# imatge-upc/rsis

Measured on AMD Instinct MI355X. Metric: training images/sec at 256x256, T=10, batch=32 per GPU, higher is better.
Workload: dtype f32

## Files before the change

rsis_amd/csrc/conv_wgrad_tiled.hip:

```cpp
#include "common.h"
#include "limb_split.h"
#include <stdlib.h>
#include <string.h>

typedef __attribute__((address_space(3))) void* lds_vp_t;
typedef __bf16 wg_bf16x8 __attribute__((ext_vector_type(8)));
typedef unsigned wg_u32x4 __attribute__((ext_vector_type(4)));

#define WG_LIMB_PRODUCTS 6
[[maybe_unused]] __device__ constexpr int wg_limb_pa[9] = {2, 1, 0, 1, 0, 0, 2, 1, 2};
[[maybe_unused]] __device__ constexpr int wg_limb_pb[9] = {0, 1, 2, 0, 1, 0, 1, 2, 2};

__device__ __forceinline__ void wg_limb_pack8(const float (&v)[8], wg_bf16x8 (&out)[3]) {
  wg_u32x4 q[3];
#pragma unroll
  for (int m = 0; m < 4; ++m) {
    float lo[3], hi[3];
    rsis_limb_split3(v[2 * m], lo[0], lo[1], lo[2]);
    rsis_limb_split3(v[2 * m + 1], hi[0], hi[1], hi[2]);
    q[0][m] = __builtin_amdgcn_perm(__float_as_uint(v[2 * m + 1]), __float_as_uint(v[2 * m]), 0x07060302u);
    q[1][m] = __builtin_amdgcn_perm(__float_as_uint(hi[1]), __float_as_uint(lo[1]), 0x07060302u);
    q[2][m] = __builtin_amdgcn_perm(__float_as_uint(hi[2]), __float_as_uint(lo[2]), 0x07060302u);
  }
#pragma unroll
  for (int l = 0; l < 3; ++l) out[l] = __builtin_bit_cast(wg_bf16x8, q[l]);
}

struct WgradTiledArgs {
  const float* dy;
  const float* x;
  float* dw;
  int B, Cs, H, W, Cout;
  int ldo, n_off, interleave_hid;
  int n_co_tiles, n_n_tiles, n_sp_tiles, tiles_per_split;
};

#define RSIS_OOB 0x7FFFFFF0u

template <int BM, int BN, int WGM, int WGN, int KS, int TW, int KSP = 1, int RAG = 0, int LIMB = 0>
__device__ __forceinline__ void wgrad_tiled_body(const WgradTiledArgs& p, const int bx, const int by) {
#if __HIP_DEVICE_COMPILE__
  constexpr int TM = BM / WGM / 32, TN = BN / WGN / 32;
  constexpr int KK = KS * KS, HALO = KS / 2;
  constexpr int TP = KS == 1 ? 32 : 64;
  constexpr int TH = TP / TW;
  constexpr int NG = TP / 4;
  constexpr int GPR = TW / 4;
  constexpr int PW = TW + 2 * HALO, PH = TH + 2 * HALO, IMS = PW * PH;
  constexpr int CI_P = KS == 1 ? BN : (BN + KK - 2) / KK + 1;
  constexpr int AS = BM * TP;
  constexpr int XS = KS == 1 ? BN * TP : (CI_P * IMS + 255) / 256 * 256;
  constexpr int NA = BM * NG / 256;
  constexpr int NB4 = KS == 1 ? BN * NG / 256 : 0;
  constexpr int NB1 = KS == 1 ? 0 : XS / 256;
  static_assert(WGM * WGN * KSP == 4 && (BM * NG) % 256 == 0 && (KS == 3 || (BN * NG) % 256 == 0) && (NG / 2) % KSP == 0 && (NG / 2 / KSP) % 2 == 0, "config");

  __shared__ __attribute__((aligned(16))) float lds[2 * (AS + XS)];
  float* const As0 = lds;
  float* const Xs0 = lds + 2 * AS;

  const int tid = threadIdx.x, lane = tid & 63, l31 = lane & 31, hi = lane >> 5;
  const int wave = __builtin_amdgcn_readfirstlane(tid >> 6);
  const int wk = wave / (WGM * WGN), wm = (wave % (WGM * WGN)) / WGN, wn = wave % WGN;
  const int H = p.H, W = p.W, HW = H * W, Cs = p.Cs, Cout = p.Cout;
  const int co_t = bx % p.n_co_tiles, n_t = bx / p.n_co_tiles;
  const int co0 = co_t * BM, n0 = n_t * BN;
  const int ci0 = n0 / KK;
  const int Nn = Cs * KK;
  const int tiles_x = RAG ? (W + TW - 1) / TW : W / TW, tiles_y = RAG ? (H + TH - 1) / TH : H / TH;
  const int rx = W - (tiles_x - 1) * TW, ry = H - (tiles_y - 1) * TH;
  const int t_begin = by * p.tiles_per_split;
  const int t_end = min(t_begin + p.tiles_per_split, p.n_sp_tiles);
  if (t_begin >= t_end) return;

  unsigned voa[NA];
#pragma unroll
  for (int i = 0; i < NA; ++i) {
    const int idx = tid + i * 256;
    const int row = idx / NG, sl = idx % NG;
    const int G = (sl & ~7) | ((sl & 7) ^ (row & 7));
    const int y = G / GPR, x4 = G % GPR;
    voa[i] = co0 + row < Cout ? ((unsigned)((co0 + row) * HW + y * W + x4 * 4) * 4u) | (RAG == 2 && x4 * 4 >= rx ? 1u : 0u) | (RAG == 2 && y >= ry ? 2u : 0u) : RSIS_OOB;
  }
  unsigned voa1[RAG == 1 ? 4 * NA : 1];
  unsigned vob1r[RAG == 1 && NB4 ? 4 * NB4 : 1];
  if constexpr (RAG == 1) {
#pragma unroll
    for (int k = 0; k < 4 * NA; ++k) {
      const int P = k * 256 + tid, idx = P >> 2, e = P & 3;
      const int row = idx / NG, sl = idx % NG;
      const int G = (sl & ~7) | ((sl & 7) ^ (row & 7));
      const int y = G / GPR, x = (G % GPR) * 4 + e;
      voa1[k] = co0 + row < Cout ? ((unsigned)((co0 + row) * HW + y * W + x) * 4u) | (x >= rx ? 1u : 0u) | (y >= ry ? 2u : 0u) : RSIS_OOB;
    }
    if constexpr (KS == 1) {
#pragma unroll
      for (int k = 0; k < 4 * NB4; ++k) {
        const int P = k * 256 + tid, idx = P >> 2, e = P & 3;
        const int row = idx / NG, sl = idx % NG;
        const int G = (sl & ~7) | ((sl & 7) ^ (row & 7));
        const int y = G / GPR, x = (G % GPR) * 4 + e;
        vob1r[k] = n0 + row < Cs ? ((unsigned)((n0 + row) * HW + y * W + x) * 4u) | (x >= rx ? 1u : 0u) | (y >= ry ? 2u : 0u) : RSIS_OOB;
      }
    }
  }
  unsigned vob4[NB4 ? NB4 : 1];
  unsigned vob1[NB1 ? NB1 : 1];
  unsigned cls1[NB1 ? NB1 : 1];
  if constexpr (KS == 1) {
#pragma unroll
    for (int i = 0; i < NB4; ++i) {
      const int idx = tid + i * 256;
      const int row = idx / NG, sl = idx % NG;
      const int G = (sl & ~7) | ((sl & 7) ^ (row & 7));
      const int y = G / GPR, x4 = G % GPR;
      vob4[i] = n0 + row < Cs ? ((unsigned)((n0 + row) * HW + y * W + x4 * 4) * 4u) | (RAG == 2 && x4 * 4 >= rx ? 1u : 0u) | (RAG == 2 && y >= ry ? 2u : 0u) : RSIS_OOB;
    }
  } else {
#pragma unroll
    for (int i = 0; i < NB1; ++i) {
      const int e = tid + i * 256;
      const int cl = e / IMS, rem = e - cl * IMS;
      const int py = rem / PW, pxx = rem - py * PW;
      const bool ok = cl < CI_P && ci0 + cl < Cs;
      vob1[i] = ok ? (unsigned)(cl * HW + py * W + pxx) * 4u : RSIS_OOB;
      cls1[i] = (py == 0 ? 1u : 0u) | (py - 1 >= ry ? 2u : 0u) | (pxx == 0 ? 4u : 0u) | (pxx - 1 >= rx ? 8u : 0u);
    }
  }

  int sg[NG / 2 / KSP];
  int bo[NG / 2 / KSP];
#pragma unroll
  for (int gg = 0; gg < NG / 2 / KSP; ++gg) {
    const int g = gg * KSP + (KSP == 1 ? 0 : wk);
    sg[gg] = ((2 * g + hi) ^ (l31 & 7)) * 4;
    bo[gg] = KS == 1 ? 0 : (g / (TW / 8)) * PW + (g % (TW / 8)) * 8;
  }
  const int arow = (wm * TM * 32 + l31) * TP;
  int xb[TN];
#pragma unroll
  for (int j = 0; j < TN; ++j) {
    const int nl = wn * TN * 32 + j * 32 + l31;
    if constexpr (KS == 1) {
      xb[j] = nl * TP;
    } else {
      const int n = n0 + nl;
      const int cl = n / KK - ci0, rs = n - (n / KK) * KK;
      xb[j] = cl * IMS + (rs / KS) * PW + (rs % KS) + 4 * hi;
    }
  }

  f32x16 acc[TM][TN];
#pragma unroll
  for (int i = 0; i < TM; ++i)
#pragma unroll
    for (int j = 0; j < TN; ++j)
#pragma unroll
      for (int r = 0; r < 16; ++r) acc[i][j][r] = 0.f;

  int tb = t_begin / (tiles_x * tiles_y);
  int trem = t_begin - tb * (tiles_x * tiles_y);
  int ty = trem / tiles_x, tx = trem - ty * tiles_x;

#define WG_ISSUE(BUF)                                                                                          \
  {                                                                                                            \
    const int y0 = ty * TH, x0 = tx * TW;                                                                      \
    const float* ab = p.dy + ((size_t)tb * Cout * HW + y0 * W + x0);                                           \
    const __amdgpu_buffer_rsrc_t ra_ = __builtin_amdgcn_make_buffer_rsrc((void*)ab, 0, 0x7FFFFFF0, 0x00020000); \
    const unsigned lastm = (tx == tiles_x - 1 ? 1u : 0u) | (ty == tiles_y - 1 ? 2u : 0u);                      \
    if constexpr (RAG == 1) {                                                                                  \
      float* As = As0 + (BUF) * AS + wave * 64;                                                                \
      _Pragma("unroll") for (int k = 0; k < 4 * NA; ++k)                                                       \
        __builtin_amdgcn_raw_ptr_buffer_load_lds(ra_, (lds_vp_t)(As + k * 256), 4, (voa1[k] & lastm) ? RSIS_OOB : (voa1[k] & ~3u), 0, 0, 0); \
    } else {                                                                                                   \
      float* As = As0 + (BUF) * AS + wave * 256;                                                               \
      _Pragma("unroll") for (int i = 0; i < NA; ++i)                                                           \
        __builtin_amdgcn_raw_ptr_buffer_load_lds(ra_, (lds_vp_t)(As + i * 1024), 16,                           \
                                                 RAG == 2 ? ((voa[i] & lastm) ? RSIS_OOB : (voa[i] & ~3u)) : voa[i], 0, 0, 0); \
    }                                                                                                          \
    if constexpr (KS == 1) {                                                                                   \
      const float* bb = p.x + ((size_t)tb * Cs * HW + y0 * W + x0);                                            \
      const __amdgpu_buffer_rsrc_t rb_ = __builtin_amdgcn_make_buffer_rsrc((void*)bb, 0, 0x7FFFFFF0, 0x00020000); \
      if constexpr (RAG == 1) {                                                                                \
        float* Xs = Xs0 + (BUF) * XS + wave * 64;                                                              \
        _Pragma("unroll") for (int k = 0; k < 4 * NB4; ++k)                                                    \
          __builtin_amdgcn_raw_ptr_buffer_load_lds(rb_, (lds_vp_t)(Xs + k * 256), 4, (vob1r[k] & lastm) ? RSIS_OOB : (vob1r[k] & ~3u), 0, 0, 0); \
      } else {                                                                                                 \
        float* Xs = Xs0 + (BUF) * XS + wave * 256;                                                             \
        _Pragma("unroll") for (int i = 0; i < NB4; ++i)                                                        \
          __builtin_amdgcn_raw_ptr_buffer_load_lds(rb_, (lds_vp_t)(Xs + i * 1024), 16,                         \
                                                   RAG == 2 ? ((vob4[i] & lastm) ? RSIS_OOB : (vob4[i] & ~3u)) : vob4[i], 0, 0, 0); \
      }                                                                                                        \
    } else {                                                                                                   \
      const float* bb = p.x + (((size_t)tb * Cs + ci0) * HW + (y0 - 1) * W + (x0 - 1));                        \
      const __amdgpu_buffer_rsrc_t rb_ = __builtin_amdgcn_make_buffer_rsrc((void*)bb, 0, 0x7FFFFFF0, 0x00020000); \
      const unsigned edge = (y0 == 0 ? 1u : 0u) | (ty == tiles_y - 1 ? 2u : 0u) | (x0 == 0 ? 4u : 0u) | (tx == tiles_x - 1 ? 8u : 0u); \
      float* Xs = Xs0 + (BUF) * XS + wave * 64;                                                                \
      _Pragma("unroll") for (int i = 0; i < NB1; ++i) {                                                        \
        const unsigned vo = (cls1[i] & edge) ? RSIS_OOB : vob1[i];                                             \
        __builtin_amdgcn_raw_ptr_buffer_load_lds(rb_, (lds_vp_t)(Xs + i * 256), 4, vo, 0, 0, 0);               \
      }                                                                                                        \
    }                                                                                                          \
    if (++tx == tiles_x) { tx = 0; if (++ty == tiles_y) { ty = 0; ++tb; } }                                    \
  }
#define WG_LAND() __builtin_amdgcn_s_waitcnt(0x0F70);

  WG_ISSUE(0)
  WG_LAND()
  __syncthreads();
  const int ntl = t_end - t_begin;
  for (int t = 0; t < ntl; ++t) {
    const int cur = t & 1;
    if (t + 1 < ntl) WG_ISSUE(cur ^ 1)
    {
      const float* As = As0 + cur * AS + arow;
      const float* Xs = Xs0 + cur * XS;
      if constexpr (LIMB) {
#pragma unroll
        for (int g = 0; g < NG / 2 / KSP; g += 2) {
          wg_bf16x8 al[TM][3], bl[TN][3];
#pragma unroll
          for (int i = 0; i < TM; ++i) {
            const f32x4 a0 = *reinterpret_cast<const f32x4*>(As + i * 32 * TP + sg[g]);
            const f32x4 a1 = *reinterpret_cast<const f32x4*>(As + i * 32 * TP + sg[g + 1]);
            const float v[8] = {a0[0], a0[1], a0[2], a0[3], a1[0], a1[1], a1[2], a1[3]};
            wg_limb_pack8(v, al[i]);
          }
#pragma unroll
          for (int j = 0; j < TN; ++j) {
            float v[8];
            if constexpr (KS == 1) {
              const f32x4 b0 = *reinterpret_cast<const f32x4*>(Xs + xb[j] + sg[g]);
              const f32x4 b1 = *reinterpret_cast<const f32x4*>(Xs + xb[j] + sg[g + 1]);
#pragma unroll
              for (int e = 0; e < 4; ++e) { v[e] = b0[e]; v[4 + e] = b1[e]; }
            } else {
#pragma unroll
              for (int u = 0; u < 2; ++u)
#pragma unroll
                for (int e = 0; e < 4; ++e)
                  v[4 * u + e] = Xs[xb[j] + (KSP == 1 ? ((g + u) / (TW / 8)) * PW + ((g + u) % (TW / 8)) * 8 : bo[g + u]) + e];
            }
            wg_limb_pack8(v, bl[j]);
          }
#pragma unroll
          for (int q = 0; q < WG_LIMB_PRODUCTS; ++q)
#pragma unroll
            for (int i = 0; i < TM; ++i)
#pragma unroll
              for (int j = 0; j < TN; ++j)
                acc[i][j] = __builtin_amdgcn_mfma_f32_32x32x16_bf16(al[i][wg_limb_pa[q]], bl[j][wg_limb_pb[q]], acc[i][j], 0, 0, 0);
        }
      } else
#pragma unroll
      for (int g = 0; g < NG / 2 / KSP; ++g) {
        f32x4 a4[TM];
#pragma unroll
        for (int i = 0; i < TM; ++i) a4[i] = *reinterpret_cast<const f32x4*>(As + i * 32 * TP + sg[g]);
        if constexpr (KS == 1) {
          f32x4 b4[TN];
#pragma unroll
          for (int j = 0; j < TN; ++j) b4[j] = *reinterpret_cast<const f32x4*>(Xs + xb[j] + sg[g]);
#pragma unroll
          for (int e = 0; e < 4; ++e)
#pragma unroll
            for (int i = 0; i < TM; ++i)
#pragma unroll
              for (int j = 0; j < TN; ++j) acc[i][j] = __builtin_amdgcn_mfma_f32_32x32x2f32(a4[i][e], b4[j][e], acc[i][j], 0, 0, 0);
        } else {
#pragma unroll
          for (int e = 0; e < 4; ++e) {
            float b[TN];
#pragma unroll
            for (int j = 0; j < TN; ++j) b[j] = Xs[xb[j] + (KSP == 1 ? (g / (TW / 8)) * PW + (g % (TW / 8)) * 8 : bo[g]) + e];
#pragma unroll
            for (int i = 0; i < TM; ++i)
#pragma unroll
              for (int j = 0; j < TN; ++j) acc[i][j] = __builtin_amdgcn_mfma_f32_32x32x2f32(a4[i][e], b[j], acc[i][j], 0, 0, 0);
          }
        }
      }
    }
    WG_LAND()
    __syncthreads();
  }
#undef WG_ISSUE
#undef WG_LAND

  const __amdgpu_buffer_rsrc_t rdw = __builtin_amdgcn_make_buffer_rsrc((void*)p.dw, 0, (unsigned)((size_t)Cout * p.ldo * 4), 0x00020000);
  const int ihid = p.interleave_hid;
  const unsigned ldb = (unsigned)p.ldo * 4u;
#pragma unroll
  for (int j = 0; j < TN; ++j) {
    const int n = n0 + wn * TN * 32 + j * 32 + l31;
    if (n >= Nn) continue;
#pragma unroll
    for (int i = 0; i < TM; ++i) {
      const int row0 = co0 + wm * TM * 32 + i * 32 + 4 * hi;
      const int rows_left = Cout - row0;
      const unsigned vo = (unsigned)((ihid > 0 ? row0 >> 2 : row0) * p.ldo + p.n_off + n) * 4u;
#pragma unroll
      for (int r = 0; r < 16; ++r) {
        const int k = (r & 3) + 8 * (r >> 2);
        const unsigned ro = (unsigned)(ihid > 0 ? (r & 3) * ihid + 2 * (r >> 2) : k) * ldb;
        __builtin_amdgcn_raw_ptr_buffer_atomic_fadd_f32(acc[i][j][r], rdw, k < rows_left ? vo + ro : 0x7FFFFFF0u, 0, 0);
      }
    }
  }
#endif
}

#define RSIS_WG_MAXJ 48
struct WgradTiledGroup {
  int n;
  int begin[RSIS_WG_MAXJ + 1];
  WgradTiledArgs job[RSIS_WG_MAXJ];
};
static_assert(sizeof(WgradTiledGroup) <= 4000, "kernel arguments are limited to 4 KB");

template <int BM, int BN, int WGM, int WGN, int KS, int TW, int KSP = 1, int RAG = 0, int LIMB = 0>
__global__ __launch_bounds__(256) void conv_wgrad_tiled_group_kernel(const WgradTiledGroup g) {
  const int b = blockIdx.x;
  int lo = 0, hi = g.n - 1;
  while (lo < hi) {
    const int mid = (lo + hi + 1) >> 1;
    if (g.begin[mid] <= b) lo = mid; else hi = mid - 1;
  }
  const WgradTiledArgs& p = g.job[lo];
  const int local = b - g.begin[lo];
  const int ntile = p.n_co_tiles * p.n_n_tiles;
  wgrad_tiled_body<BM, BN, WGM, WGN, KS, TW, KSP, RAG, LIMB>(p, local % ntile, local / ntile);
}

static unsigned wg_limb_mask(int ks, int tw) {
  if (ks == 3) return tw == 16 ? 0x3Fu : (tw == 8 ? 1u << 5 : 0u);
  return tw == 16 || tw == 8 ? 1u << 2 : 0u;
}
static bool wg_use_limbs(int ks, int tw, int code, int rag) {
  static const int mode = [] {
    const char* e = getenv("RSIS_WGRAD_LIMBS");
    if (!e || !e[0]) return 0;
    if (e[0] == '0') return 1;
    return strcmp(e, "all") == 0 ? 2 : 0;
  }();
  if (mode) return mode == 2;
  return rag == 0 && ((wg_limb_mask(ks, tw) >> code) & 1u);
}

static int tiled_tw(int H, int W, int ks) {
  const int tp = ks == 1 ? 32 : 64;
  for (int tw = ks == 1 ? 32 : 16; tw >= 8; tw >>= 1)
    if (W % tw == 0 && H % (tp / tw) == 0) return tw;
  return 0;
}
static int tiled_tw_ragged(int W, int ks) {
  const int wide = ks == 1 ? 32 : 16;
  return W > 16 ? wide : (W > 8 ? 16 : 8);
}

static int tiled_cfg_code(const WgradTiledArgs& a, int ks) {
  const int nmod = (a.Cs * ks * ks) % 128;
  const bool narrow = nmod != 0 && nmod <= 64;
  if (ks == 1 && a.Cout > 32) return 2;
  if (a.Cout <= 32) return narrow && !rsis_deterministic() ? 0 : 1;
  if (a.Cout <= 64) return narrow ? 2 : 3;
  return narrow ? 4 : 5;
}

static void tiled_split_plan(WgradTiledArgs* jobs, int n, int ks, bool big_tile, bool alone, int rag) {
  if (alone && rag == 0) {
    WgradTiledArgs& a = jobs[0];
    const int ntile = a.n_co_tiles * a.n_n_tiles;
    const int slots = ks == 1 ? (big_tile ? 256 : 512) : 256 * (big_tile ? 2 : 3);
    int nsplit = ntile >= slots ? 1 : slots / ntile;
    if (nsplit > a.n_sp_tiles / 2) nsplit = a.n_sp_tiles / 2;
    if (nsplit < 1 || rsis_deterministic()) nsplit = 1;
    a.tiles_per_split = rsis_cdiv(a.n_sp_tiles, nsplit);
    return;
  }
  long total_iters = 0;
  for (int j = 0; j < n; ++j) total_iters += (long)jobs[j].n_co_tiles * jobs[j].n_n_tiles * jobs[j].n_sp_tiles;
  static const int env_tb = getenv("RSIS_WG_GROUP_BLOCKS") ? atoi(getenv("RSIS_WG_GROUP_BLOCKS")) : 0;
  const long target_blocks = env_tb > 0 ? env_tb : 2048;
  long L = (total_iters + target_blocks - 1) / target_blocks;
  if (L < 2) L = 2;
  if (rsis_deterministic()) L = 1L << 40;
  for (int j = 0; j < n; ++j) {
    int nsplit = rsis_cdiv(jobs[j].n_sp_tiles, L);
    if (nsplit < 1) nsplit = 1;
    jobs[j].tiles_per_split = rsis_cdiv(jobs[j].n_sp_tiles, nsplit);
  }
}

template <int BM, int BN, int WGM, int WGN, int KS, int TW, int KSP = 1, int RAG = 0, int LIMB = 0>
static int launch_group_cfg(WgradTiledArgs* jobs, int n, bool alone, hipStream_t st) {
  constexpr int TH = (KS == 1 ? 32 : 64) / TW;
  for (int j = 0; j < n; ++j) {
    WgradTiledArgs& a = jobs[j];
    a.n_co_tiles = rsis_cdiv(a.Cout, BM);
    a.n_n_tiles = rsis_cdiv((long)a.Cs * KS * KS, BN);
    a.n_sp_tiles = RAG ? a.B * rsis_cdiv(a.H, TH) * rsis_cdiv(a.W, TW) : a.B * (a.H / TH) * (a.W / TW);
  }
  tiled_split_plan(jobs, n, KS, BM * BN >= 128 * 128, alone, RAG);
  for (int j0 = 0; j0 < n; j0 += RSIS_WG_MAXJ) {
    WgradTiledGroup g;
    g.n = n - j0 < RSIS_WG_MAXJ ? n - j0 : RSIS_WG_MAXJ;
    int blocks = 0;
    for (int j = 0; j < g.n; ++j) {
      const WgradTiledArgs& a = jobs[j0 + j];
      g.begin[j] = blocks;
      g.job[j] = a;
      blocks += a.n_co_tiles * a.n_n_tiles * rsis_cdiv(a.n_sp_tiles, a.tiles_per_split);
    }
    g.begin[g.n] = blocks;
    hipLaunchKernelGGL((conv_wgrad_tiled_group_kernel<BM, BN, WGM, WGN, KS, TW, KSP, RAG, LIMB>), dim3(blocks), dim3(256), 0, st, g);
    if (rsis_check_launch() != RSIS_OK) return RSIS_ERR_LAUNCH;
  }
  return RSIS_OK;
}

template <int KS, int TW, int RAG, int LIMB>
static int launch_group_code(int code, WgradTiledArgs* jobs, int n, bool alone, hipStream_t st) {
  switch (code) {
    case 0: return launch_group_cfg<32, 64, 1, 2, KS, TW, 2, RAG, LIMB>(jobs, n, alone, st);
    case 1: return launch_group_cfg<32, 128, 1, 4, KS, TW, 1, RAG, LIMB>(jobs, n, alone, st);
    case 2: return launch_group_cfg<64, 64, 2, 2, KS, TW, 1, RAG, LIMB>(jobs, n, alone, st);
    case 3: return launch_group_cfg<64, 128, 2, 2, KS, TW, 1, RAG, LIMB>(jobs, n, alone, st);
    case 4: return launch_group_cfg<128, 64, 2, 2, KS, TW, 1, RAG, LIMB>(jobs, n, alone, st);
    default: return launch_group_cfg<128, 128, 2, 2, KS, TW, 1, RAG, LIMB>(jobs, n, alone, st);
  }
}

template <int KS, int TW>
static int launch_group_tw(int rag, int code, WgradTiledArgs* jobs, int n, bool alone, hipStream_t st) {
  const bool limb = wg_use_limbs(KS, TW, code, rag);
  switch (rag * 2 + limb) {
    case 0: return launch_group_code<KS, TW, 0, 0>(code, jobs, n, alone, st);
    case 1: return launch_group_code<KS, TW, 0, 1>(code, jobs, n, alone, st);
    case 2: return launch_group_code<KS, TW, 1, 0>(code, jobs, n, alone, st);
    case 3: return launch_group_code<KS, TW, 1, 1>(code, jobs, n, alone, st);
    case 4: return launch_group_code<KS, TW, 2, 0>(code, jobs, n, alone, st);
    default: return launch_group_code<KS, TW, 2, 1>(code, jobs, n, alone, st);
  }
}

static int launch_group(int ks, int tw, int rag, int code, WgradTiledArgs* jobs, int n, bool alone, hipStream_t st) {
  if (ks == 1 && tw == 32) return launch_group_tw<1, 32>(rag, code, jobs, n, alone, st);
  if (ks == 1 && tw == 16) return launch_group_tw<1, 16>(rag, code, jobs, n, alone, st);
  if (ks == 1 && tw == 8) return launch_group_tw<1, 8>(rag, code, jobs, n, alone, st);
  if (ks == 3 && tw == 16) return launch_group_tw<3, 16>(rag, code, jobs, n, alone, st);
  if (ks == 3 && tw == 8) return launch_group_tw<3, 8>(rag, code, jobs, n, alone, st);
  return RSIS_ERR_ARG;
}

static WgradTiledArgs tiled_args(const WgradArgs& w) {
  WgradTiledArgs a = {};
  a.dy = w.dy; a.x = w.x; a.dw = w.dw; a.B = w.B; a.Cs = w.Cs; a.H = w.H; a.W = w.W; a.Cout = w.Cout;
  a.ldo = w.ldo; a.n_off = w.n_off; a.interleave_hid = w.interleave_hid;
  return a;
}

static int tiled_launch_jobs(const WgradArgs* w, int n, int ks, bool alone, hipStream_t st) {
  if (n < 1) return RSIS_OK;
  WgradTiledArgs* all = (WgradTiledArgs*)malloc(sizeof(WgradTiledArgs) * n * 2);
  int* key = (int*)malloc(sizeof(int) * n);
  if (!all || !key) { free(all); free(key); return RSIS_ERR_LAUNCH; }
  WgradTiledArgs* bucket = all + n;
  for (int j = 0; j < n; ++j) {
    WgradTiledArgs& a = all[j] = tiled_args(w[j]);
    const int twa = tiled_tw(a.H, a.W, ks);
    if (twa) key[j] = twa * 8 + tiled_cfg_code(a, ks);
    else {
      if (ks == 1 && (a.H * a.W) % 4 == 0) { a.W = a.H * a.W; a.H = 1; }
      key[j] = (a.W % 4 == 0 ? 2048 : 1024) + tiled_tw_ragged(a.W, ks) * 8 + tiled_cfg_code(a, ks);
    }
  }
  int rc = RSIS_OK;
  for (int j = 0; j < n && rc == RSIS_OK; ++j) {
    if (key[j] < 0) continue;
    const int k = key[j];
    int m = 0;
    for (int i = j; i < n; ++i)
      if (key[i] == k) { bucket[m++] = all[i]; key[i] = -1; }
    rc = launch_group(ks, (k & 1023) / 8, k >> 10, k % 8, bucket, m, alone, st);
  }
  free(all); free(key);
  return rc;
}

int rsis_launch_conv_wgrad_tiled_group(const WgradArgs* w, int n, int ks, hipStream_t st) { return tiled_launch_jobs(w, n, ks, false, st); }
int rsis_launch_conv_wgrad_tiled(const WgradArgs& w, int ks, hipStream_t st) { return tiled_launch_jobs(&w, 1, ks, true, st); }

bool rsis_wgrad_tiled_supported(const WgradArgs& w, int ks) {
  if (!(ks == 1 || ks == 3) || w.stride != 1 || w.pad != ks / 2 || w.H != w.Ho || w.W != w.Wo) return false;
  static const bool ragged_on = !(getenv("RSIS_WGRAD_RAGGED") && getenv("RSIS_WGRAD_RAGGED")[0] == '0');
  if (tiled_tw(w.H, w.W, ks) == 0 && !ragged_on) return false;
  const long img = (long)w.H * w.W * 4;
  return (long)w.Cout * img < (1L << 30) && (long)w.Cs * img < (1L << 30);
}
```

Before: 941.9.

## Add XCD-aware block remapping and wider tile selection for grouped wgrad

Grouped weight-gradient launches can now remap block indices so that consecutive logical blocks land on the same XCD, aiming to improve L2 reuse of shared dy/x tiles across the MI355X's chiplets. Grouped 1x1 convolutions with large Cout/Cs are moved to the 128x128 tile config, and limb-split bf16 math is enabled for that config. Each behaviour is selected by a per-config mask and can be overridden with environment variables. Risks include load imbalance from the new block order and lower occupancy or precision differences with the larger limb-based tiles.

```diff
diff --git a/rsis_amd/csrc/conv_wgrad_tiled.hip b/rsis_amd/csrc/conv_wgrad_tiled.hip
--- a/rsis_amd/csrc/conv_wgrad_tiled.hip
+++ b/rsis_amd/csrc/conv_wgrad_tiled.hip
@@ -1,5 +1,6 @@
 #include "common.h"
 #include "limb_split.h"
+#include "wgrad_block_order.h"
 #include <stdlib.h>
 #include <string.h>
 
@@ -313,6 +314,7 @@
 #define RSIS_WG_MAXJ 48
 struct WgradTiledGroup {
   int n;
+  int xcd_order;
   int begin[RSIS_WG_MAXJ + 1];
   WgradTiledArgs job[RSIS_WG_MAXJ];
 };
@@ -320,7 +322,7 @@
 
 template <int BM, int BN, int WGM, int WGN, int KS, int TW, int KSP = 1, int RAG = 0, int LIMB = 0>
 __global__ __launch_bounds__(256) void conv_wgrad_tiled_group_kernel(const WgradTiledGroup g) {
-  const int b = blockIdx.x;
+  const int b = g.xcd_order ? rsis_xcd_logical_block(blockIdx.x, gridDim.x) : (int)blockIdx.x;
   int lo = 0, hi = g.n - 1;
   while (lo < hi) {
     const int mid = (lo + hi + 1) >> 1;
@@ -334,7 +336,7 @@
 
 static unsigned wg_limb_mask(int ks, int tw) {
   if (ks == 3) return tw == 16 ? 0x3Fu : (tw == 8 ? 1u << 5 : 0u);
-  return tw == 16 || tw == 8 ? 1u << 2 : 0u;
+  return (tw == 16 || tw == 8 ? 1u << 2 : 0u) | 1u << 5;
 }
 static bool wg_use_limbs(int ks, int tw, int code, int rag) {
   static const int mode = [] {
@@ -347,6 +349,22 @@
   return rag == 0 && ((wg_limb_mask(ks, tw) >> code) & 1u);
 }
 
+static unsigned wg_xcd_mask(int ks, int tw) {
+  if (ks == 3) return tw == 16 ? 0x5u : 0u;
+  return tw == 32 ? 1u << 5 : 0u;
+}
+static int wg_xcd_order(int ks, int tw, int code, int rag) {
+  static const int mode = [] {
+    const char* e = getenv("RSIS_WGRAD_XCD");
+    if (!e || !e[0]) return 0;
+    if (e[0] == '0') return 1;
+    return strcmp(e, "all") == 0 ? 2 : 0;
+  }();
+  if (mode) return mode == 2;
+  return rag == 0 && ((wg_xcd_mask(ks, tw) >> code) & 1u);
+}
+static constexpr int tiled_code_of(int bm, int bn) { return bm == 32 ? (bn == 64 ? 0 : 1) : (bm == 64 ? (bn == 64 ? 2 : 3) : (bn == 64 ? 4 : 5)); }
+
 static int tiled_tw(int H, int W, int ks) {
   const int tp = ks == 1 ? 32 : 64;
   for (int tw = ks == 1 ? 32 : 16; tw >= 8; tw >>= 1)
@@ -358,13 +376,37 @@
   return W > 16 ? wide : (W > 8 ? 16 : 8);
 }
 
-static int tiled_cfg_code(const WgradTiledArgs& a, int ks) {
+static int tiled_cfg_code_single(const WgradTiledArgs& a, int ks) {
   const int nmod = (a.Cs * ks * ks) % 128;
   const bool narrow = nmod != 0 && nmod <= 64;
   if (ks == 1 && a.Cout > 32) return 2;
   if (a.Cout <= 32) return narrow && !rsis_deterministic() ? 0 : 1;
   if (a.Cout <= 64) return narrow ? 2 : 3;
   return narrow ? 4 : 5;
+}
+
+static int wg_job_class(const WgradTiledArgs& a, int ks) {
+  if (ks == 1) return a.Cout <= 32 ? -1 : (a.Cout >= 128 && a.Cs >= 128 ? 1 : 0);
+  const int nmod = (a.Cs * ks * ks) % 128;
+  if (nmod == 0 || nmod > 64) return -1;
+  return a.Cout <= 32 ? 0 : (a.Cout <= 64 ? 1 : 2);
+}
+static int wg_wide_code(int ks, int cls) { return ks == 1 ? 5 : 2 * cls + 1; }
+static int wg_group_tile(int ks, int tw, int cls) {
+  return ks == 1 && cls == 1 && (tw == 32 || tw == 16) ? 5 : -1;
+}
+static int tiled_cfg_code(const WgradTiledArgs& a, int ks, int tw, bool grouped) {
+  static const int mode = [] {
+    const char* e = getenv("RSIS_WGRAD_TILES");
+    if (!e || !e[0]) return 0;
+    if (strcmp(e, "0") == 0) return 1;
+    return strcmp(e, "wide") == 0 ? 2 : 0;
+  }();
+  const int single = tiled_cfg_code_single(a, ks);
+  const int cls = wg_job_class(a, ks);
+  if (!grouped || cls < 0 || mode == 1 || rsis_deterministic()) return single;
+  const int code = mode == 2 ? wg_wide_code(ks, cls) : wg_group_tile(ks, tw, cls);
+  return code < 0 ? single : code;
 }
 
 static void tiled_split_plan(WgradTiledArgs* jobs, int n, int ks, bool big_tile, bool alone, int rag) {
@@ -404,6 +446,7 @@
   tiled_split_plan(jobs, n, KS, BM * BN >= 128 * 128, alone, RAG);
   for (int j0 = 0; j0 < n; j0 += RSIS_WG_MAXJ) {
     WgradTiledGroup g;
+    g.xcd_order = !alone && wg_xcd_order(KS, TW, tiled_code_of(BM, BN), RAG);
     g.n = n - j0 < RSIS_WG_MAXJ ? n - j0 : RSIS_WG_MAXJ;
     int blocks = 0;
     for (int j = 0; j < g.n; ++j) {
@@ -469,10 +512,10 @@
   for (int j = 0; j < n; ++j) {
     WgradTiledArgs& a = all[j] = tiled_args(w[j]);
     const int twa = tiled_tw(a.H, a.W, ks);
-    if (twa) key[j] = twa * 8 + tiled_cfg_code(a, ks);
+    if (twa) key[j] = twa * 8 + tiled_cfg_code(a, ks, twa, !alone);
     else {
       if (ks == 1 && (a.H * a.W) % 4 == 0) { a.W = a.H * a.W; a.H = 1; }
-      key[j] = (a.W % 4 == 0 ? 2048 : 1024) + tiled_tw_ragged(a.W, ks) * 8 + tiled_cfg_code(a, ks);
+      key[j] = (a.W % 4 == 0 ? 2048 : 1024) + tiled_tw_ragged(a.W, ks) * 8 + tiled_cfg_code_single(a, ks);
     }
   }
   int rc = RSIS_OK;
diff --git a/rsis_amd/csrc/wgrad_block_order.h b/rsis_amd/csrc/wgrad_block_order.h
--- /dev/null
+++ b/rsis_amd/csrc/wgrad_block_order.h
@@ -0,0 +1,12 @@
+#pragma once
+
+#if defined(__HIPCC__) || defined(__CUDACC__)
+#define RSIS_ORDER_HD __host__ __device__
+#else
+#define RSIS_ORDER_HD
+#endif
+
+RSIS_ORDER_HD inline int rsis_xcd_logical_block(const int b, const int n) {
+  const int x = b & 7, q = n >> 3, r = n & 7;
+  return x * q + (x < r ? x : r) + (b >> 3);
+}
```

Result: faster. 957.9, median of 6 (+1.7%).
